# shijun18/H-DenseFormer

Measured on AMD Instinct MI355X. Metric: train samples/sec on 4x128^3 volumes, higher is better.
Workload: dtype bf16

## Files before the change

### h-denseformer_amd/csrc/head_ops.hip

```cpp
#include "unet_ops_internal.h"

namespace {

constexpr int HEAD_MAXCLS = 8;

template <typename T, int MC>
__global__ __launch_bounds__(256) void head_fwd_kernel(const T* __restrict__ in, int64_t in_pitch,
                                                       const float* __restrict__ scale, const float* __restrict__ shift,
                                                       const float* __restrict__ w, const float* __restrict__ b,
                                                       T* __restrict__ logits, int N, int C, int ncls, int64_t vox,
                                                       int per, int vec4) {
  HDF_LIGHT_PRIO();
  constexpr int EPC = ST<T>::EPC;
  extern __shared__ float outs[];
  float* part = outs + MC * per;
  const int n = blockIdx.y;
  const int cols = C / EPC;
  const bool pow2 = (cols & (cols - 1)) == 0 && cols <= 64;
  const int vlanes = 256 / cols;
  const int col = threadIdx.x % cols, vl = min((int)threadIdx.x / cols, vlanes - 1);
  const bool lane_on = (int)threadIdx.x < vlanes * cols;
  const int c0 = col * EPC;
  float sc[EPC], sh[EPC], wv[MC][EPC];
#pragma unroll
  for (int e = 0; e < EPC; e++) {
    sc[e] = scale ? scale[(int64_t)n * C + c0 + e] : 1.f;
    sh[e] = scale ? shift[(int64_t)n * C + c0 + e] : 0.f;
#pragma unroll
    for (int o = 0; o < MC; o++) wv[o][e] = (o < ncls) ? w[min(o, ncls - 1) * C + c0 + e] : 0.f;
  }
  const int64_t vb = (int64_t)blockIdx.x * per, ve = min(vox, vb + per);
  constexpr int U = 4;
  const int iters = (per + U * vlanes - 1) / (U * vlanes);
  for (int it = 0; it < iters; it++) {
    const int64_t v0 = vb + vl + (int64_t)it * U * vlanes;
    float f[U][EPC];
#pragma unroll
    for (int u = 0; u < U; u++) {
      const int64_t v = min(v0 + (int64_t)u * vlanes, ve - 1);
      load_chunk<T>(in + ((int64_t)n * vox + v) * in_pitch + c0, f[u]);
    }
#pragma unroll
    for (int u = 0; u < U; u++) {
      float acc[MC];
#pragma unroll
      for (int o = 0; o < MC; o++) acc[o] = 0.f;
#pragma unroll
      for (int e = 0; e < EPC; e++) {
        float x = f[u][e];
        if (scale) x = fmaxf(x * sc[e] + sh[e], 0.f);
#pragma unroll
        for (int o = 0; o < MC; o++) acc[o] += x * wv[o][e];
      }
      if (pow2) {
        for (int off = 1; off < cols; off <<= 1) {
#pragma unroll
          for (int o = 0; o < MC; o++) acc[o] += __shfl_xor(acc[o], off, 64);
        }
      } else {
        __syncthreads();
#pragma unroll
        for (int o = 0; o < MC; o++) part[threadIdx.x * MC + o] = acc[o];
        __syncthreads();
        if (col == 0) {
          for (int k = 1; k < cols; k++)
#pragma unroll
            for (int o = 0; o < MC; o++) acc[o] += part[(threadIdx.x + k) * MC + o];
        }
      }
      const int64_t lv = v0 + (int64_t)u * vlanes - vb;
      if (col == 0 && lane_on && lv < per) {
#pragma unroll
        for (int o = 0; o < MC; o++) outs[o * per + (int)lv] = acc[o];
      }
    }
  }
  __syncthreads();
  for (int o = 0; o < ncls; o++) {
    const float bo = b[o];
    if (vec4) {
      for (int lv = threadIdx.x * 4; lv < per; lv += 1024)
        if (vb + lv < vox)
          ST<T>::st4(logits + ((int64_t)n * ncls + o) * vox + vb + lv, outs[o * per + lv] + bo, outs[o * per + lv + 1] + bo,
                     outs[o * per + lv + 2] + bo, outs[o * per + lv + 3] + bo);
    } else {
      for (int lv = threadIdx.x; lv < per; lv += 256)
        if (vb + lv < vox) ST<T>::st(logits + ((int64_t)n * ncls + o) * vox + vb + lv, outs[o * per + lv] + bo);
    }
  }
}

constexpr int HEAD_VOX_MAX = 2048;
inline int head_vox(int64_t vox, int wgs = 128) {
  return (int)std::max<int64_t>(64, std::min<int64_t>(HEAD_VOX_MAX, (vox / wgs) & ~63));
}
template <typename T, int MC, bool ACC>
__global__ __launch_bounds__(256, (MC == 4 && sizeof(T) == 2) ? 4 : 1) void head_bwd_kernel(const T* __restrict__ dlogits, const T* __restrict__ in,
                                                       int64_t in_pitch, const float* __restrict__ scale,
                                                       const float* __restrict__ shift, const float* __restrict__ w,
                                                       T* __restrict__ dx, int64_t dx_pitch,
                                                       float* __restrict__ dw, float* __restrict__ db, int N, int C,
                                                       int ncls, int64_t vox, int per,
                                                       const float* __restrict__ in_mean,
                                                       const float* __restrict__ in_rstd,
                                                       float* __restrict__ inb_partials, int vec4) {
  HDF_LIGHT_PRIO();
  constexpr int EPC = 4;
  extern __shared__ float red[];
  const int n = blockIdx.y;
  const int cols = C / EPC;
  const int vlanes = 256 / cols;
  const int col = threadIdx.x % cols, vl = threadIdx.x / cols;
  const int c0 = col * EPC;
  float sc[EPC], sh[EPC], wv[MC][EPC], accw[MC][EPC], accb[MC];
  float mu[EPC], rs[EPC], s1[EPC], s2[EPC];
#pragma unroll
  for (int e = 0; e < EPC; e++) {
    sc[e] = scale ? scale[(int64_t)n * C + c0 + e] : 1.f;
    sh[e] = scale ? shift[(int64_t)n * C + c0 + e] : 0.f;
    mu[e] = inb_partials ? in_mean[(int64_t)n * C + c0 + e] : 0.f;
    rs[e] = inb_partials ? in_rstd[(int64_t)n * C + c0 + e] : 0.f;
    s1[e] = s2[e] = 0.f;
  }
#pragma unroll
  for (int o = 0; o < MC; o++) {
    accb[o] = 0.f;
#pragma unroll
    for (int e = 0; e < EPC; e++) {
      wv[o][e] = (o < ncls) ? w[min(o, ncls - 1) * C + c0 + e] : 0.f;
      accw[o][e] = 0.f;
    }
  }
  const int64_t vb = (int64_t)blockIdx.x * per, ve = min(vox, vb + per);
  if (vec4) {
    for (int i = threadIdx.x; i < MC * (per >> 2); i += 256) {
      const int o = i / (per >> 2), lv = (i - o * (per >> 2)) * 4;
      float v[4];
      ST<T>::ld4(dlogits + ((int64_t)n * ncls + min(o, ncls - 1)) * vox + min(vb + lv, vox - 4), v);
#pragma unroll
      for (int j = 0; j < 4; j++) red[(lv + j) * MC + o] = (o < ncls && vb + lv < vox) ? v[j] : 0.f;
    }
  } else {
    for (int o = 0; o < MC; o++) {
      const T* src = dlogits + ((int64_t)n * ncls + min(o, ncls - 1)) * vox;
      for (int lv = threadIdx.x; lv < per; lv += 256) {
        const float v = ST<T>::ld(src + min(vb + lv, vox - 1));
        red[lv * MC + o] = (o < ncls && vb + lv < vox) ? v : 0.f;
      }
    }
  }
  __syncthreads();
  if (vl < vlanes) {
    constexpr int U = sizeof(T) == 2 ? 2 : 4;
    for (int64_t v0 = vb + vl; v0 < ve; v0 += (int64_t)U * vlanes) {
      float f[U][EPC], g[ACC ? U : 1][EPC], dl[U][MC];
      int64_t row[U];
#pragma unroll
      for (int u = 0; u < U; u++) {
        const int64_t v = min(v0 + (int64_t)u * vlanes, ve - 1);
        row[u] = (int64_t)n * vox + v;
        ST<T>::ld4(in + row[u] * in_pitch + c0, f[u]);
        if (ACC) ST<T>::ld4(dx + row[u] * dx_pitch + c0, g[ACC ? u : 0]);
#pragma unroll
        for (int o = 0; o < MC; o++) dl[u][o] = red[(int)(v - vb) * MC + o];
      }
#pragma unroll
      for (int u = 0; u < U; u++) {
        const bool live = v0 + (int64_t)u * vlanes < ve;
#pragma unroll
        for (int o = 0; o < MC; o++) dl[u][o] = live ? dl[u][o] : 0.f;
        float d[EPC];
#pragma unroll
        for (int e = 0; e < EPC; e++) {
          float x = f[u][e];
          if (scale) x = fmaxf(x * sc[e] + sh[e], 0.f);
          float t = ACC ? g[ACC ? u : 0][e] : 0.f;
#pragma unroll
          for (int o = 0; o < MC; o++) {
            t += dl[u][o] * wv[o][e];
            accw[o][e] += dl[u][o] * x;
          }
          d[e] = t;
        }
        if (live) ST<T>::st4(dx + row[u] * dx_pitch + c0, d[0], d[1], d[2], d[3]);
        if (inb_partials) {
#pragma unroll
          for (int e = 0; e < EPC; e++) {
            const float gg = (live && f[u][e] * sc[e] + sh[e] > 0.f) ? storage_round<T>(d[e]) : 0.f;
            s1[e] += gg;
            s2[e] += gg * ((f[u][e] - mu[e]) * rs[e]);
          }
        }
        if (col == 0) {
#pragma unroll
          for (int o = 0; o < MC; o++) accb[o] += dl[u][o];
        }
      }
    }
  }
  __syncthreads();
  const int ld = (C + 1) * MC;
  if (vl < vlanes) {
#pragma unroll
    for (int o = 0; o < MC; o++) {
#pragma unroll
      for (int e = 0; e < EPC; e++) red[vl * ld + (c0 + e) * MC + o] = accw[o][e];
      if (col == 0) red[vl * ld + C * MC + o] = accb[o];
    }
  }
  __syncthreads();
  for (int i = threadIdx.x; i < (C + 1) * MC; i += 256) {
    const int c = i / MC, o = i - c * MC;
    if (o >= ncls) continue;
    float t = 0.f;
    for (int k = 0; k < vlanes; k++) t += red[k * ld + i];
    if (c < C)
      atomicAdd(dw + o * C + c, t);
    else
      atomicAdd(db + o, t);
  }
  if (inb_partials) {
    __syncthreads();
    if (vl < vlanes) {
#pragma unroll
      for (int e = 0; e < EPC; e++) {
        red[(vl * C + c0 + e) * 2 + 0] = s1[e];
        red[(vl * C + c0 + e) * 2 + 1] = s2[e];
      }
    }
    __syncthreads();
    for (int i = threadIdx.x; i < C * 2; i += 256) {
      float t = 0.f;
      for (int k = 0; k < vlanes; k++) t += red[k * C * 2 + i];
      inb_partials[((int64_t)n * gridDim.x + blockIdx.x) * C * 2 + i] = t;
    }
  }
}

}

static int allow_big_lds(const void* kern, size_t bytes) {
  if (bytes <= 64 * 1024) return HDF_OK;
  hipError_t e = hipFuncSetAttribute(kern, hipFuncAttributeMaxDynamicSharedMemorySize, 160 * 1024);
  if (e != hipSuccess) {
    hdf_set_error("hipFuncSetAttribute(MaxDynamicSharedMemorySize) failed: %s", hipGetErrorString(e));
    return HDF_ERR_HIP;
  }
  return HDF_OK;
}

int hdf_launch_head_fwd(int dtype, CRows in, NormStats ins, const float* w, const float* b, void* logits, int N, int C,
                        int ncls, int64_t vox, hipStream_t st) {
  HDF_CHECK_ARG(ncls <= HEAD_MAXCLS, "head: n_cls=%d > %d", ncls, HEAD_MAXCLS);
  HDF_CHECK_ARG(C % 16 == 0 && C <= 1024, "head_fwd: C=%d", C);
  const int per = head_vox(vox, 1024) >= 256 ? head_vox(vox, 1024) : head_vox(vox);
  const unsigned gx = (unsigned)ceil_div64(vox, per);
  const int vec4 = (vox % 4 == 0 && (reinterpret_cast<uintptr_t>(logits) & 15) == 0) ? 1 : 0;
  HDF_DISPATCH_T(dtype, {
    auto go = [&](auto kern, int mc) -> int {
      const size_t shm = (size_t)mc * (per + 256) * sizeof(float);
      HDF_TRY(allow_big_lds((const void*)kern, shm));
      hipLaunchKernelGGL(kern, dim3(gx, N), dim3(256), shm, st, (const T*)in.p, in.pitch, ins.scale, ins.shift, w, b,
                         (T*)logits, N, C, ncls, vox, per, vec4);
      return HDF_OK;
    };
    if (ncls <= 4)
      HDF_TRY(go(head_fwd_kernel<T, 4>, 4));
    else
      HDF_TRY(go(head_fwd_kernel<T, 8>, 8));
  });
  HDF_LAUNCH_CHECK();
  return HDF_OK;
}

int hdf_head_bwd_blocks(int64_t vox) { return (int)ceil_div64(vox, head_vox(vox)); }

int hdf_launch_head_bwd(int dtype, const void* dlogits, CRows in, NormStats ins, const float* w, HeadGrads g, int N, int C,
                        int ncls, int64_t vox, hipStream_t st) {
  HDF_CHECK_ARG(ncls <= HEAD_MAXCLS, "head: n_cls=%d > %d", ncls, HEAD_MAXCLS);
  HDF_CHECK_ARG(C % 16 == 0 && C <= 1024, "head_bwd: C=%d", C);
  HDF_CHECK_ARG(g.inb_partials == nullptr || (ins.scale && ins.mean && ins.rstd),
                "head_bwd: IN partials need the layer's statistics");
  const int per = head_vox(vox);
  const unsigned gx = (unsigned)hdf_head_bwd_blocks(vox);
  const int vec4 = (vox % 4 == 0 && (reinterpret_cast<uintptr_t>(dlogits) & 15) == 0) ? 1 : 0;
  HDF_DISPATCH_T(dtype, {
    const int cols = C / 4, vlanes = 256 / cols;
    const int mc = ncls <= 4 ? 4 : 8;
    const size_t shm =
        std::max(std::max((size_t)vlanes * (C + 1) * mc, (size_t)per * mc), (size_t)vlanes * C * 2) * sizeof(float);
    auto go = [&](auto kern) -> int {
      HDF_TRY(allow_big_lds((const void*)kern, shm));
      hipLaunchKernelGGL(kern, dim3(gx, N), dim3(256), shm, st, (const T*)dlogits, (const T*)in.p, in.pitch, ins.scale,
                         ins.shift, w, (T*)g.dx.p, g.dx.pitch, g.dw, g.db, N, C, ncls, vox, per, ins.mean, ins.rstd,
                         g.inb_partials, vec4);
      return HDF_OK;
    };
    if (mc == 4)
      HDF_TRY(g.accumulate_dx ? go(head_bwd_kernel<T, 4, true>) : go(head_bwd_kernel<T, 4, false>));
    else
      HDF_TRY(g.accumulate_dx ? go(head_bwd_kernel<T, 8, true>) : go(head_bwd_kernel<T, 8, false>));
  });
  HDF_LAUNCH_CHECK();
  return HDF_OK;
}
```

Baseline: 184.4.

## Software-pipeline head backward row loads and transpose dlogits staging layout

The head backward kernel now issues the first batch of input/dx row loads before staging dlogits into shared memory. Inside the main loop it prefetches the next iteration's rows as raw registers while computing the current ones, so global-load latency overlaps with the LDS fill and the arithmetic. The dlogits staging changes to a class-major shared layout with batched 16-byte vector stores, and 64-bit row indexing is replaced with 32-bit offsets from a per-block base, guarded by a new pitch check. Tail stores now write a duplicate of the first row instead of branching, which costs extra registers and relies on a hand-placed waitcnt.

Result: no change. 185.2, median of 6 (+0.5%).

```diff
diff --git a/h-denseformer_amd/csrc/head_ops.hip b/h-denseformer_amd/csrc/head_ops.hip
--- a/h-denseformer_amd/csrc/head_ops.hip
+++ b/h-denseformer_amd/csrc/head_ops.hip
@@ -3,6 +3,17 @@
 namespace {
 
 constexpr int HEAD_MAXCLS = 8;
+
+template <typename T>
+using raw4_t = std::conditional_t<sizeof(T) == 2, u32x2, f32x4>;
+template <typename T>
+__device__ __forceinline__ raw4_t<T> ld_raw4(const T* p) {
+  return *reinterpret_cast<const raw4_t<T>*>(p);
+}
+template <typename T>
+__device__ __forceinline__ void cvt_raw4(const raw4_t<T>& r, float* f) {
+  ST<T>::ld4(reinterpret_cast<const T*>(&r), f);
+}
 
 template <typename T, int MC>
 __global__ __launch_bounds__(256) void head_fwd_kernel(const T* __restrict__ in, int64_t in_pitch,
@@ -106,7 +117,7 @@
                                                        float* __restrict__ inb_partials, int vec4) {
   HDF_LIGHT_PRIO();
   constexpr int EPC = 4;
-  extern __shared__ float red[];
+  extern __shared__ __align__(16) float red[];
   const int n = blockIdx.y;
   const int cols = C / EPC;
   const int vlanes = 256 / cols;
@@ -131,42 +142,77 @@
       accw[o][e] = 0.f;
     }
   }
-  const int64_t vb = (int64_t)blockIdx.x * per, ve = min(vox, vb + per);
+  const int64_t vb = (int64_t)blockIdx.x * per;
+  const int nv = (int)(min(vox, vb + per) - vb);
+  const T* inb = in + ((int64_t)n * vox + vb) * in_pitch + c0;
+  T* dxb = dx + ((int64_t)n * vox + vb) * dx_pitch + c0;
+  constexpr int U = sizeof(T) == 2 ? 2 : 4;
+  const int step = U * vlanes;
+  const int ip = (int)in_pitch, dp = (int)dx_pitch;
+  raw4_t<T> fr[U], gr[ACC ? U : 1];
+  auto request = [&](int l0) {
+#pragma unroll
+    for (int u = 0; u < U; u++) {
+      const int lv = min(l0 + u * vlanes, nv - 1);
+      fr[u] = ld_raw4<T>(inb + lv * ip);
+      if (ACC) gr[ACC ? u : 0] = ld_raw4<T>(dxb + lv * dp);
+    }
+  };
+  request(vl);
   if (vec4) {
-    for (int i = threadIdx.x; i < MC * (per >> 2); i += 256) {
-      const int o = i / (per >> 2), lv = (i - o * (per >> 2)) * 4;
-      float v[4];
-      ST<T>::ld4(dlogits + ((int64_t)n * ncls + min(o, ncls - 1)) * vox + min(vb + lv, vox - 4), v);
-#pragma unroll
-      for (int j = 0; j < 4; j++) red[(lv + j) * MC + o] = (o < ncls && vb + lv < vox) ? v[j] : 0.f;
+    constexpr int B = 8;
+    const int q = per >> 2, tot = MC * q;
+    for (int i0 = threadIdx.x; i0 < tot; i0 += 256 * B) {
+      raw4_t<T> r[B];
+#pragma unroll
+      for (int k = 0; k < B; k++) {
+        const int i = min(i0 + k * 256, tot - 1), o = i / q, lv = (i - o * q) * 4;
+        r[k] = ld_raw4<T>(dlogits + ((int64_t)n * ncls + min(o, ncls - 1)) * vox + min(vb + lv, vox - 4));
+      }
+#pragma unroll
+      for (int k = 0; k < B; k++) {
+        const int i = i0 + k * 256, o = i / q, lv = (i - o * q) * 4;
+        float v[4];
+        cvt_raw4<T>(r[k], v);
+        const bool on = o < ncls && vb + lv < vox;
+        if (i < tot)
+          *reinterpret_cast<f32x4*>(red + o * per + lv) =
+              f32x4{on ? v[0] : 0.f, on ? v[1] : 0.f, on ? v[2] : 0.f, on ? v[3] : 0.f};
+      }
     }
   } else {
-    for (int o = 0; o < MC; o++) {
-      const T* src = dlogits + ((int64_t)n * ncls + min(o, ncls - 1)) * vox;
-      for (int lv = threadIdx.x; lv < per; lv += 256) {
-        const float v = ST<T>::ld(src + min(vb + lv, vox - 1));
-        red[lv * MC + o] = (o < ncls && vb + lv < vox) ? v : 0.f;
-      }
-    }
-  }
+    for (int lv = threadIdx.x; lv < per; lv += 256) {
+      float v[MC];
+#pragma unroll
+      for (int o = 0; o < MC; o++)
+        v[o] = ST<T>::ld(dlogits + ((int64_t)n * ncls + min(o, ncls - 1)) * vox + min(vb + lv, vox - 1));
+#pragma unroll
+      for (int o = 0; o < MC; o++) red[o * per + lv] = (o < ncls && vb + lv < vox) ? v[o] : 0.f;
+    }
+  }
+  __builtin_amdgcn_s_waitcnt(0x0f70);
   __syncthreads();
   if (vl < vlanes) {
-    constexpr int U = sizeof(T) == 2 ? 2 : 4;
-    for (int64_t v0 = vb + vl; v0 < ve; v0 += (int64_t)U * vlanes) {
-      float f[U][EPC], g[ACC ? U : 1][EPC], dl[U][MC];
-      int64_t row[U];
+    for (int l0 = vl; l0 < nv; l0 += step) {
+      float f[U][EPC], g[ACC ? U : 1][EPC], dl[U][MC], d0[EPC];
+      int row[U];
 #pragma unroll
       for (int u = 0; u < U; u++) {
-        const int64_t v = min(v0 + (int64_t)u * vlanes, ve - 1);
-        row[u] = (int64_t)n * vox + v;
-        ST<T>::ld4(in + row[u] * in_pitch + c0, f[u]);
-        if (ACC) ST<T>::ld4(dx + row[u] * dx_pitch + c0, g[ACC ? u : 0]);
-#pragma unroll
-        for (int o = 0; o < MC; o++) dl[u][o] = red[(int)(v - vb) * MC + o];
-      }
+        row[u] = min(l0 + u * vlanes, nv - 1);
+        cvt_raw4<T>(fr[u], f[u]);
+        if (ACC) cvt_raw4<T>(gr[ACC ? u : 0], g[ACC ? u : 0]);
+#pragma unroll
+        for (int o = 0; o < MC; o++) dl[u][o] = red[o * per + row[u]];
+#pragma unroll
+        for (int e = 0; e < EPC; e++) {
+          asm volatile("" : "+v"(f[u][e]));
+          if (ACC) asm volatile("" : "+v"(g[ACC ? u : 0][e]));
+        }
+      }
+      request(l0 + step);
 #pragma unroll
       for (int u = 0; u < U; u++) {
-        const bool live = v0 + (int64_t)u * vlanes < ve;
+        const bool live = l0 + u * vlanes < nv;
 #pragma unroll
         for (int o = 0; o < MC; o++) dl[u][o] = live ? dl[u][o] : 0.f;
         float d[EPC];
@@ -182,7 +228,12 @@
           }
           d[e] = t;
         }
-        if (live) ST<T>::st4(dx + row[u] * dx_pitch + c0, d[0], d[1], d[2], d[3]);
+        if (u == 0) {
+#pragma unroll
+          for (int e = 0; e < EPC; e++) d0[e] = d[e];
+        }
+        ST<T>::st4(dxb + (live ? row[u] : row[0]) * dp, live ? d[0] : d0[0], live ? d[1] : d0[1], live ? d[2] : d0[2],
+                   live ? d[3] : d0[3]);
         if (inb_partials) {
 #pragma unroll
           for (int e = 0; e < EPC; e++) {
@@ -279,6 +330,8 @@
                         int ncls, int64_t vox, hipStream_t st) {
   HDF_CHECK_ARG(ncls <= HEAD_MAXCLS, "head: n_cls=%d > %d", ncls, HEAD_MAXCLS);
   HDF_CHECK_ARG(C % 16 == 0 && C <= 1024, "head_bwd: C=%d", C);
+  HDF_CHECK_ARG(in.pitch < (1 << 20) && g.dx.pitch < (1 << 20), "head_bwd: row pitch %lld / %lld", (long long)in.pitch,
+                (long long)g.dx.pitch);
   HDF_CHECK_ARG(g.inb_partials == nullptr || (ins.scale && ins.mean && ins.rstd),
                 "head_bwd: IN partials need the layer's statistics");
   const int per = head_vox(vox);
```
